# FermiQ/octree-mg

Hardware: AMD Instinct MI355X
Metric: V-cycle cell-updates/s + smoother HBM GB/s vs roofline, 3D Poisson 512^3 (higher is better)
Workload: dtype f64; 1 GPU; C3: 3D Poisson, 512^3 per GPU, box 16, periodic, GSRB FAS V-cycle (n_cycle_down=up=2); mode=weak, box_size=16, parallelism=domain-decomposition x1 (RCCL halos)

## Files before the change

### octree-mg_amd/csrc/omg_tiles.hip

```cpp
#include <stdexcept>
#include <string>

#include "omg_face.h"
#include "omg_gsrb.h"
#include "omg_kernels.h"

namespace omg {

constexpr int kPsBS16 = 512, kPsWaves = 8;
constexpr int kSumsLPW = 32, kSumsR = 4;
constexpr bool kSumsNT = true, kSubNTLd = false, kSubNTSt = false;

template <int NC, int OP, int BS, bool STORE = true>
__device__ __forceinline__ void resid_restrict_core(const LevelView& F, const LevelView& Cv, double lambda,
                                                    unsigned long long* maxbits, int restrict_on,
                                                    const int* parent_local, const int* dixp, int b, double* sb,
                                                    const v2d* fr);

template <int NC, int OP, int BS, bool STORE = true>
__device__ __forceinline__ void resid_restrict_box(const LevelView& F, const LevelView& Cv, double lambda,
                                                   unsigned long long* maxbits, int restrict_on,
                                                   const int* parent_local, const int* dixp, int b, double* sb,
                                                   const double* __restrict__ rsh = nullptr, int n_rsh = 0) {
  using TL = Tl<NC>;
  constexpr int NST = TL::NST, HV = TL::HV, NR = (HV + BS - 1) / BS;
  const int tid = threadIdx.x;
  const long long boff = (long long)b * F.stride;
  const double* __restrict__ u = F.phi + boff;
  const double* __restrict__ f = F.data + F.vstride + boff;
  for (int q = tid; q < NST / 2; q += BS) reinterpret_cast<v2d*>(sb)[q] = ld_nt(u + 2 * q);
  v2d fr[NR];
#pragma unroll
  for (int r = 0; r < NR; r++) {
    const int q2 = tid + BS * r;
    if (q2 < HV) fr[r] = ld_nt(f + 2 * q2);
  }
  if (n_rsh) {
    const RhsSub rsub(rsh, n_rsh);
#pragma unroll
    for (int r = 0; r < NR; r++)
      if (tid + BS * r < HV) {
        double a = fr[r].x, b2 = fr[r].y;
        rsub(a, b2);
        fr[r].x = a;
        fr[r].y = b2;
      }
  }
  __syncthreads();
  resid_restrict_core<NC, OP, BS, STORE>(F, Cv, lambda, maxbits, restrict_on, parent_local, dixp, b, sb, fr);
}

template <bool ON>
__device__ __forceinline__ int step_zero(double mx) {
  if constexpr (ON) {
    int zero = 0;
    asm volatile("" : "+v"(zero) : "v"(mx));
    return zero;
  } else {
    return 0;
  }
}

template <int NC, int OP, int BS, bool STORE>
__device__ __forceinline__ void resid_restrict_core(const LevelView& F, const LevelView& Cv, double lambda,
                                                    unsigned long long* maxbits, int restrict_on,
                                                    const int* parent_local, const int* dixp, int b, double* sb,
                                                    const v2d* fr) {
  using TL = Tl<NC>;
  constexpr int HV = TL::HV, FH = TL::FH, FS = TL::FS, NR = (HV + BS - 1) / BS, HN = NC / 2;
  const int tid = threadIdx.x;
  double* __restrict__ res = F.data + 3 * F.vstride + (long long)b * F.stride;

  const OpCoef<OP> K(F, lambda);
  double mx = 0.0;
  double2 rv[NR];
#pragma unroll
  for (int r = 0; r < NR; r++) {
    const int q2 = tid + BS * r;
    if (q2 >= HV) continue;
    const int e = q2 >= HV / 2, o = 1 - e;
    Nbr7 s0, s1;
    if constexpr (HN % 2 == 0) {
      pair_stencil<NC>(sb + o * HV, sb + 2 * HV + o * FH, FS, e,
                       2 * q2 - e * HV + step_zero<!STORE && (NR > 1)>(mx), s0, s1);
    } else {
      int i, j, k;
      TL::decode(2 * q2, i, j, k);
      s0.xm = sb[TL::ocell(i - 1, j, k)]; s0.xp = sb[TL::ocell(i + 1, j, k)];
      s0.ym = sb[TL::ocell(i, j - 1, k)]; s0.yp = sb[TL::ocell(i, j + 1, k)];
      s0.zm = sb[TL::ocell(i, j, k - 1)]; s0.zp = sb[TL::ocell(i, j, k + 1)];
      TL::decode(2 * q2 + 1, i, j, k);
      s1.xm = sb[TL::ocell(i - 1, j, k)]; s1.xp = sb[TL::ocell(i + 1, j, k)];
      s1.ym = sb[TL::ocell(i, j - 1, k)]; s1.yp = sb[TL::ocell(i, j + 1, k)];
      s1.zm = sb[TL::ocell(i, j, k - 1)]; s1.zp = sb[TL::ocell(i, j, k + 1)];
    }
    const double2 cc = reinterpret_cast<const double2*>(sb)[q2];
    s0.c = cc.x;
    s1.c = cc.y;
    double l0, l1;
    op_pair<NC, OP>(K, F, b, e, 2 * q2 - e * HV, s0, s1, l0, l1);
    const double r0 = fr[r].x - l0, r1 = fr[r].y - l1;
    mx = amax(mx, amax(fabs(r0), fabs(r1)));
    rv[r] = make_double2(r0, r1);
    if constexpr (STORE) st_nt(res + 2 * q2, r0, r1);
  }
  if (maxbits) launch_max<BS>(maxbits, mx);
  if (!restrict_on || parent_local[b] < 0) return;

  const int pb = parent_local[b], dp = dixp[b];
  const int dx = dp & 1023, dy = (dp >> 10) & 1023, dz = dp >> 20;
  const long long poff = (long long)pb * Cv.stride;
  for (int pass = 0; pass < 2; pass++) {
    double* __restrict__ dst = pass == 0 ? Cv.phi + poff : Cv.data + 3 * Cv.vstride + poff;
    for (int q = tid; q < HN * HN * HN; q += BS) {
      const int i = q % HN + 1, j = (q / HN) % HN + 1, k = q / (HN * HN) + 1;
      double acc = 0.0;
#pragma unroll
      for (int kk = 0; kk < 2; kk++)
#pragma unroll
        for (int jj = 0; jj < 2; jj++)
#pragma unroll
          for (int ii = 0; ii < 2; ii++) acc += sb[TL::oint(2 * i - 1 + ii, 2 * j - 1 + jj, 2 * k - 1 + kk)];
      dst[off_int(Cv, dx + i, dy + j, dz + k)] = 0.125 * acc;
    }
    if (pass == 0) {
      __syncthreads();
#pragma unroll
      for (int r = 0; r < NR; r++) {
        const int q2 = tid + BS * r;
        if (q2 < HV) reinterpret_cast<double2*>(sb)[q2] = rv[r];
      }
      __syncthreads();
    }
  }
}

template <int NC, int OP, int BS, bool STORE = true>
__global__ void __launch_bounds__(BS) k_resid_restrict(LevelView F, LevelView Cv, double lambda,
                                                       unsigned long long* maxbits, int restrict_on,
                                                       const int* parent_local, const int* dixp,
                                                       const int* list, const double* __restrict__ rsh,
                                                       int n_rsh) {
  __shared__ double sb[Tl<NC>::NST];
  const int q = xcd_box(blockIdx.x, gridDim.x, F.rev);
  resid_restrict_box<NC, OP, BS, STORE>(F, Cv, lambda, maxbits, restrict_on, parent_local, dixp,
                                        list ? list[q] : q, sb, rsh, n_rsh);
}

template <int NC>
__device__ __forceinline__ int sr_int(int d, int v, int a, int c) {
  return d == 0 ? Tl<NC>::oint(v, a, c) : (d == 1 ? Tl<NC>::oint(a, v, c) : Tl<NC>::oint(a, c, v));
}
template <int NC>
__device__ __forceinline__ int sr_edge(int d, int t, bool lo, int nl, int a, int c) {
  const int t1 = d == 0 ? 1 : 0, t2 = d == 2 ? 1 : 2, ax = t == 0 ? t1 : t2;
  const int fn = 2 * ax + (lo ? 1 : 2);
  const int i = d == 0 ? nl : a, j = d == 1 ? nl : (d == 0 ? a : c), k = d == 2 ? nl : c;
  return ax == 0 ? Tl<NC>::ogh(fn, j, k) : (ax == 1 ? Tl<NC>::ogh(fn, i, k) : Tl<NC>::ogh(fn, i, j));
// ... 433 lines not shown
  }
  __syncthreads();
  const RbSide rbs{Cv, nullptr, rbgv, rbgv ? 1 : 0};
  gsrb_box<NC, OP, BS, 2, true, RB>(F, lambda, 1, 2, bc, nullptr, nullptr, b, lds, nullptr, RB ? &rbs : nullptr);
}

template <int NC, int OP, int BS, bool RB = false>
__global__ void __launch_bounds__(BS, RB ? 4 : kPsWaves) k_prolong_smooth(LevelView Cv, LevelView F, double lambda,
                                                       const int* parent_local, const int* dixp, GcBC bc,
                                                       int one_child, const int* list, const uint8_t* push0,
                                                       double* rbgv) {
  __shared__ double lds[prolong_smooth_lds<NC>()];
  const int t = xcd_box(blockIdx.x, gridDim.x, F.rev);
  prolong_smooth_box<NC, OP, BS, RB>(Cv, F, lambda, parent_local, dixp, bc, one_child, push0, list ? list[t] : t,
                                     lds, rbgv);
}

void launch_prolong_smooth(const LevelView& C, const LevelView& F, int op, double lambda, const int* parent_local,
                           const int* dixp, const GcBC& bc, int one_child, const int* list, int n_list,
                           const uint8_t* push0, hipStream_t st, bool rb, double* rbgv) {
  const int n = list ? n_list : F.n;
  if (n == 0) return;
  const dim3 g(n);
  if (rb) {
    if (F.nc != 16 && F.nc != 8) throw std::runtime_error("launch_prolong_smooth: refinement boundaries need 16^3 / 8^3");
#define OMG_PSR(NC, BS)                                                                                         \
  if (op == OP_HELM)                                                                                            \
    k_prolong_smooth<NC, OP_HELM, BS, true><<<g, BS, 0, st>>>(C, F, lambda, parent_local, dixp, bc, one_child, \
                                                              list, push0, rbgv);                               \
  else                                                                                                          \
    k_prolong_smooth<NC, OP_LPL, BS, true><<<g, BS, 0, st>>>(C, F, lambda, parent_local, dixp, bc, one_child,  \
                                                             list, push0, rbgv);
    if (F.nc == 16) OMG_PSR(16, kPsBS16) else OMG_PSR(8, 256)
#undef OMG_PSR
    return;
  }
#define OMG_PS(NC, BS)                                                                                \
  if (op == OP_HELM)                                                                                  \
    k_prolong_smooth<NC, OP_HELM, BS><<<g, BS, 0, st>>>(C, F, lambda, parent_local, dixp, bc, one_child, \
                                                        list, push0, nullptr);                        \
  else                                                                                                \
    k_prolong_smooth<NC, OP_LPL, BS><<<g, BS, 0, st>>>(C, F, lambda, parent_local, dixp, bc, one_child,  \
                                                       list, push0, nullptr);
  switch (F.nc) {
    case 16: OMG_PS(16, kPsBS16) break;
    case 8: OMG_PS(8, 256) break;
    case 4: OMG_PS(4, 256) break;
    default: OMG_PS(2, 256) break;
  }
#undef OMG_PS
}

template <bool NT>
__device__ __forceinline__ double2 sums_ld(const double* p) {
  if (NT) {
    const v2d t = ld_nt(p);
    return make_double2(t.x, t.y);
  }
  return *reinterpret_cast<const double2*>(p);
}
template <bool NT>
__device__ __forceinline__ void sums_st(double* p, double2 v) {
  if (NT)
    st_nt(p, v.x, v.y);
  else
    *reinterpret_cast<double2*>(p) = v;
}

template <int NC, bool SUB, bool SH = SUB, int LPW = kSumsLPW>
__global__ void __launch_bounds__(64) k_box_sums3(LevelView L, int iv, const int* __restrict__ leaves,
                                                  int n_leaves, double* __restrict__ out,
                                                  const double* __restrict__ shifts, int n_sh) {
  constexpr int H = NC / 2, R = kSumsR < NC ? kSumsR : NC, SEG = R * H;
  constexpr bool NTL = SUB ? kSubNTLd : kSumsNT;
  constexpr int CH2 = SEG;
  constexpr int PER = LPW * CH2 / 64;
  constexpr int P = 2 * SEG + 1;
  constexpr int NCH = NC * NC / R;
  __shared__ double lds[LPW * P];
  const int lane = threadIdx.x, b0 = (L.rev ? gridDim.x - 1 - blockIdx.x : blockIdx.x) * LPW;
  const long long hv = L.hv;
  double* src[PER];
  int dst[PER];
  bool own[PER];
#pragma unroll
  for (int r = 0; r < PER; r++) {
    const int t = lane + 64 * r, bb = t / CH2, w = t % CH2, seg = w / (SEG / 2), off = w % (SEG / 2);
    const int q = min(b0 + bb, n_leaves - 1);
    own[r] = b0 + bb < n_leaves;
    src[r] = boxp(L, iv, leaves[q]) + seg * hv + 2 * off;
    dst[r] = bb * P + seg * SEG + 2 * off;
  }
  static_assert(SH || !SUB, "k_box_sums3: the storing form subtracts");
  const RhsSub rsub(shifts, SH ? n_sh : 0);
  double2 va[PER], vb[PER];
  auto chunk_off = [](int c) { return H * (((c % (NC / R)) * R) + NC * (c / (NC / R))); };
#pragma unroll
  for (int r = 0; r < PER; r++) va[r] = sums_ld<NTL>(src[r]);
#pragma unroll
  for (int r = 0; r < PER; r++) vb[r] = sums_ld<NTL>(src[r] + chunk_off(1));
  double acc = 0.0;
  const double* my = lds + lane * P;
  auto process = [&](double2* v, int c) {
    __syncthreads();
    const int rc = chunk_off(c);
#pragma unroll
    for (int r = 0; r < PER; r++) {
      if (SH) rsub(v[r].x, v[r].y);
      if (SUB && own[r]) sums_st<kSubNTSt>(src[r] + rc, v[r]);
      lds[dst[r]] = v[r].x;
      lds[dst[r] + 1] = v[r].y;
    }
    __syncthreads();
    if (c + 2 < NCH) {
      const int r2 = chunk_off(c + 2);
#pragma unroll
      for (int r = 0; r < PER; r++) v[r] = sums_ld<NTL>(src[r] + r2);
    }
    const int k = c / (NC / R) + 1, j0 = (c % (NC / R)) * R + 1;
    if (lane < LPW) {
#pragma unroll
      for (int rr = 0; rr < R; rr++) {
        const int ca = (1 + j0 + rr + k) & 1;
        const double* A = my + ca * SEG + rr * H;
        const double* B = my + (1 - ca) * SEG + rr * H;
#pragma unroll
        for (int q = 0; q < H; q++) {
          acc += A[q];
          acc += B[q];
        }
      }
    }
  };
  static_assert(NCH % 2 == 0, "chunks come in pairs");
  for (int c = 0; c < NCH; c += 2) {
    process(va, c);
    process(vb, c + 1);
  }
  if (out && lane < LPW && b0 + lane < n_leaves) out[b0 + lane] = acc;
}

__global__ void __launch_bounds__(64) k_box_sums_any(LevelView L, int iv, const int* leaves, int n_leaves,
                                                     double* out) {
  const int q = blockIdx.x * 64 + threadIdx.x;
  if (q >= n_leaves) return;
  const double* u = boxp(L, iv, leaves[q]);
  double acc = 0.0;
  for (int k = 1; k <= L.nc; k++)
    for (int j = 1; j <= L.nc; j++)
      for (int i = 1; i <= L.nc; i++) acc += u[off_int(L, i, j, k)];
  out[q] = acc;
}

__global__ void __launch_bounds__(64) k_seq_sum3(const double* __restrict__ box_sums, int n, double w,
                                                 double* __restrict__ acc, int init) {
  constexpr int CH = 1024, PL = CH / 128, G = 16;
  __shared__ double st[CH];
  const int lane = threadIdx.x;
  double a = init ? 0.0 : *acc;
  double2 pre[PL];
  auto fetch = [&](int base) {
#pragma unroll
    for (int r = 0; r < PL; r++) {
      const int q = base + 2 * (lane + 64 * r);
      pre[r].x = q < n ? box_sums[q] : 0.0;
      pre[r].y = q + 1 < n ? box_sums[q + 1] : 0.0;
    }
  };
  fetch(0);
  for (int base = 0; base < n; base += CH) {
    __syncthreads();
#pragma unroll
    for (int r = 0; r < PL; r++) reinterpret_cast<double2*>(st)[lane + 64 * r] = pre[r];
    __syncthreads();
    if (base + CH < n) fetch(base + CH);
    const int m = min(CH, n - base);
    if (m == CH) {
      double cur[G], nxt[G];
#pragma unroll
      for (int t = 0; t < G; t++) cur[t] = st[t];
      for (int g = 0; g < CH / G; g++) {
        const int gn = g + 1 < CH / G ? g + 1 : g;
#pragma unroll
        for (int t = 0; t < G; t++) nxt[t] = st[G * gn + t];
        double p[G];
#pragma unroll
        for (int t = 0; t < G; t++) p[t] = w * cur[t];
#pragma unroll
        for (int t = 0; t < G; t++) a = a + p[t];
#pragma unroll
        for (int t = 0; t < G; t++) cur[t] = nxt[t];
      }
    } else {
      for (int q = 0; q < m; q++) a = a + w * st[q];
    }
  }
  if (lane == 0) *acc = a;
}

template <int NC, int BS>
__global__ void __launch_bounds__(BS) k_fill_tile(LevelView L, GcBC bc, double* sendbuf) {
  constexpr int HV = Tl<NC>::HV;
  __shared__ double sb[2 * HV];
  const int b = xcd_box(blockIdx.x, gridDim.x, L.rev);
  const FaceTopo T = load_topo(L, b);
  const double* u = L.phi + (long long)b * L.stride;
  for (int q = threadIdx.x; q < HV; q += BS) reinterpret_cast<v2d*>(sb)[q] = reinterpret_cast<const v2d*>(u)[q];
  __syncthreads();
  tile_face_fill<NC>(L, b, T, sb, 3, bc, sendbuf);
}

template <int NC, int BS>
__global__ void __launch_bounds__(BS) k_fill_tile_xl(LevelView L, GcBC bc, double* sendbuf,
                                                     const double* __restrict__ xl) {
  using TL = Tl<NC>;
  constexpr int HV = TL::HV, H = NC / 2, FH = H * NC;
  __shared__ double sb[2 * HV];
  const int b = xcd_box(blockIdx.x, gridDim.x, L.rev);
  const FaceTopo T = load_topo(L, b);
  const double* u = L.phi + (long long)b * L.stride;
  bool phys = false;
#pragma unroll
  for (int nb = 0; nb < 6; nb++) phys |= T.kind(nb) == NB_PHYS;
  if (phys) {
    for (int q = threadIdx.x; q < HV; q += BS) reinterpret_cast<v2d*>(sb)[q] = reinterpret_cast<const v2d*>(u)[q];
  } else {
    const int t = threadIdx.x;
    for (int q = t; q < 2 * FH; q += BS) {
      const int e = q / FH, w = q % FH, pl = w / (FH / 2), r2 = w % (FH / 2);
      const int off = e * HV + (pl ? FH * (NC - 1) : 0) + 2 * r2;
      *reinterpret_cast<v2d*>(sb + off) = *reinterpret_cast<const v2d*>(u + off);
    }
    for (int q = t; q < 4 * NC * (H / 2); q += BS) {
      const int r2 = q % (H / 2), row = q / (H / 2), k = row % NC, jj = (row / NC) & 1, e = row / (2 * NC);
      const int off = e * HV + H * ((jj ? NC - 1 : 0) + NC * k) + 2 * r2;
      *reinterpret_cast<v2d*>(sb + off) = *reinterpret_cast<const v2d*>(u + off);
    }
    const double* xb = xl + (long long)b * 512;
    for (int q = t; q < 2 * NC * NC; q += BS) {
      const int f = q / (NC * NC), c = q % (NC * NC), j = c % NC + 1, k = c / NC + 1;
      sb[TL::oint(f ? NC : 1, j, k)] = xb[q];
    }
  }
  __syncthreads();
  tile_face_fill<NC>(L, b, T, sb, 3, bc, sendbuf);
}

void launch_fill_tile_xl(const LevelView& L, const GcBC& bc, double* sendbuf, const double* xl, hipStream_t st) {
  if (L.n == 0) return;
  if (L.nc != 16) throw std::runtime_error("launch_fill_tile_xl: 16^3 boxes only");
  k_fill_tile_xl<16, 512><<<L.n, 512, 0, st>>>(L, bc, sendbuf, xl);
}

bool launch_fill_tile(const LevelView& L, const GcBC& bc, double* sendbuf, hipStream_t st) {
  if (L.n == 0) return true;
  const dim3 g(L.n);
  switch (L.nc) {
    case 16: k_fill_tile<16, 512><<<g, 512, 0, st>>>(L, bc, sendbuf); return true;
    case 8: k_fill_tile<8, 256><<<g, 256, 0, st>>>(L, bc, sendbuf); return true;
    case 4: k_fill_tile<4, 64><<<g, 64, 0, st>>>(L, bc, sendbuf); return true;
    default: return false;
  }
}

bool launch_smooth_resid(const LevelView& F, const LevelView& C, int op, double lambda, int restrict_on,
                         const int* parent_local, const int* dixp, hipStream_t st, const int* list,
                         int n_list, const GcBC& bc, bool has_rb, bool has_phys, const double* rbgv) {
  if (op != OP_LPL && op != OP_HELM) return false;
  if (!has_rb) rbgv = nullptr;
  const int n = list ? n_list : F.n;
  if (n == 0) return true;
  const dim3 g(n);
#define OMG_SR_RB(NC, BS, RB)                                                                                    \
  if (op == OP_LPL)                                                                                              \
    k_smooth_resid<NC, OP_LPL, BS, RB><<<g, BS, 0, st>>>(F, C, lambda, restrict_on, parent_local, dixp, list, bc,   \
                                                         rbgv);                                                   \
  else                                                                                                           \
    k_smooth_resid<NC, OP_HELM, BS, RB><<<g, BS, 0, st>>>(F, C, lambda, restrict_on, parent_local, dixp, list, bc,  \
                                                          rbgv);
#define OMG_SR(NC, BS)           \
  if (has_rb) {                  \
    OMG_SR_RB(NC, BS, 2)         \
  } else if (has_phys) {         \
    OMG_SR_RB(NC, BS, 1)         \
  } else {                       \
    OMG_SR_RB(NC, BS, 0)         \
  }
  switch (F.nc) {
    case 16: OMG_SR(16, 512) return true;
    case 8: OMG_SR(8, 256) return true;
    default: return false;
  }
#undef OMG_SR
#undef OMG_SR_RB
}

bool tiled_nc(int nc) { return nc == 16 || nc == 8 || nc == 4 || nc == 2; }

void launch_resid_restrict(const LevelView& F, const LevelView& C, int op, double lambda,
                           unsigned long long* maxbits, int restrict_on, const int* parent_local,
                           const int* dixp, hipStream_t st, const int* list, int n_list, RhsShifts rs,
                           bool store) {
  const int n = list ? n_list : F.n;
  if (n == 0) return;
  if (rs.n < 0 || rs.n > kRhsPendMax || (rs.n && !rs.s))
    throw std::runtime_error("launch_resid_restrict: at most kRhsPendMax pending rhs shifts");
  const dim3 g(n);
#define OMG_RR_OP(NC, BS, OPV)                                                                             \
  if (store)                                                                                               \
    k_resid_restrict<NC, OPV, BS, true><<<g, dim3(BS), 0, st>>>(F, C, lambda, maxbits, restrict_on,        \
                                                                parent_local, dixp, list, rs.s, rs.n);     \
  else                                                                                                     \
    k_resid_restrict<NC, OPV, BS, false><<<g, dim3(BS), 0, st>>>(F, C, lambda, maxbits, restrict_on,       \
                                                                 parent_local, dixp, list, rs.s, rs.n);
#define OMG_RR(NC, BS) OMG_FOR_OP(op, OMG_RR_OP, NC, BS)
  switch (F.nc) {
    case 16: OMG_RR(16, 512) break;
    case 8: OMG_RR(8, 256) break;
    case 4: OMG_RR(4, 256) break;
    default: OMG_RR(2, 256) break;
  }
#undef OMG_RR
#undef OMG_RR_OP
}

void launch_prolong_fill(const LevelView& C, const LevelView& F, int iv, const int* parent_local,
                         const int* dixp, const GcBC& bc, double* sendbuf, bool sub, bool skip1,
                         hipStream_t st, const int* list, int n_list, bool save_old, const RBRec* rb) {
  const int n = list ? n_list : F.n;
  if (n == 0) return;
  const dim3 g(n);
  const int so = save_old && !skip1;
#define OMG_PF(NC, BS)                                                                                              \
  if (rb && sub)                                                                                                    \
    k_prolong_fill<NC, BS, true, true><<<g, BS, 0, st>>>(C, F, iv, parent_local, dixp, bc, sendbuf, skip1, list, so, rb); \
  else if (rb)                                                                                                      \
    k_prolong_fill<NC, BS, false, true><<<g, BS, 0, st>>>(C, F, iv, parent_local, dixp, bc, sendbuf, skip1, list, so, rb); \
  else if (sub)                                                                                                     \
    k_prolong_fill<NC, BS, true><<<g, BS, 0, st>>>(C, F, iv, parent_local, dixp, bc, sendbuf, skip1, list, so, rb); \
  else                                                                                                              \
    k_prolong_fill<NC, BS, false><<<g, BS, 0, st>>>(C, F, iv, parent_local, dixp, bc, sendbuf, skip1, list, so, rb);
  switch (F.nc) {
    case 16: OMG_PF(16, 512) break;
    case 8: OMG_PF(8, 256) break;
    case 4: OMG_PF(4, 256) break;
    default: OMG_PF(2, 256) break;
  }
#undef OMG_PF
}

template <int NC, int OP, int BS, bool NT = false>
// ... 79 lines not shown
      sb[TL::ogh(nb, a, c)] = C.phi[(long long)T.arg(f) * C.stride + sr_int<NC>(d, low ? NC : 1, a, c)];
    }
    const double* __restrict__ res = C.data + 3 * C.vstride + boff;
#pragma unroll
    for (int r = 0; r < NR; r++) {
      const int q2 = tid + BS * r;
      if (q2 < HV) rr[r] = ld_nt(res + 2 * q2);
    }
  }
  __syncthreads();
  tile_face_fill<NC>(C, b, T, sb, 3, bc, nullptr);
  if (!par) return;
  if (T.nonlocal()) {
    for (int p = tid; p < 6 * NC * NC; p += BS) {
      const int f = p / (NC * NC), cell = p % (NC * NC);
      if (T.kind(f) != NB_PHYS) continue;
      const int nb = f + 1, a = cell % NC + 1, c = cell / NC + 1, d = f >> 1;
      const bool low = nb & 1;
      const int gi = TL::ogh(nb, a, c);
      sb[gi] = phys_ghost(C, bc, b, (long long)b * 6 + f, nb, T.phys_code(f), a, c, gi,
                          sb[sr_int<NC>(d, low ? 1 : NC, a, c)], sb[sr_int<NC>(d, low ? 2 : NC - 1, a, c)]);
    }
  }
  __syncthreads();
  double* __restrict__ old = C.data + 2 * C.vstride + boff;
  double* __restrict__ rhs = C.data + C.vstride + boff;
  for (int q = tid; q < NST / 2; q += BS) {
    const v2d x = reinterpret_cast<const v2d*>(sb)[q];
    st_nt(old + 2 * q, x.x, x.y);
  }
  const OpCoef<OP> K(C, lambda);
  constexpr int FS = TL::FS;
#pragma unroll
  for (int r = 0; r < NR; r++) {
    const int q2 = tid + BS * r;
    if (q2 >= HV) continue;
    const int e = q2 >= HV / 2, o = 1 - e;
    Nbr7 s0, s1;
    if constexpr (H % 2 == 0) {
      pair_stencil<NC>(sb + o * HV, sb + 2 * HV + o * FH, FS, e, 2 * q2 - e * HV, s0, s1);
    } else {
      int i, j, k;
      TL::decode(2 * q2, i, j, k);
      s0.xm = sb[TL::ocell(i - 1, j, k)]; s0.xp = sb[TL::ocell(i + 1, j, k)];
      s0.ym = sb[TL::ocell(i, j - 1, k)]; s0.yp = sb[TL::ocell(i, j + 1, k)];
      s0.zm = sb[TL::ocell(i, j, k - 1)]; s0.zp = sb[TL::ocell(i, j, k + 1)];
      TL::decode(2 * q2 + 1, i, j, k);
      s1.xm = sb[TL::ocell(i - 1, j, k)]; s1.xp = sb[TL::ocell(i + 1, j, k)];
      s1.ym = sb[TL::ocell(i, j - 1, k)]; s1.yp = sb[TL::ocell(i, j + 1, k)];
      s1.zm = sb[TL::ocell(i, j, k - 1)]; s1.zp = sb[TL::ocell(i, j, k + 1)];
    }
    const double2 cc = reinterpret_cast<const double2*>(sb)[q2];
    s0.c = cc.x;
    s1.c = cc.y;
    double l0, l1;
    op_pair<NC, OP>(K, C, b, e, 2 * q2 - e * HV, s0, s1, l0, l1);
    st_nt(rhs + 2 * q2, l0 + rr[r].x, l1 + rr[r].y);
  }
}

void launch_fill_crhs(const LevelView& C, int op, double lambda, const GcBC& bc, const uint8_t* parmask,
                      hipStream_t st) {
  if (C.n == 0) return;
  const dim3 g(C.n);
#define OMG_FC_OP(NC, BS, OPV) k_fill_crhs<NC, OPV, BS><<<g, BS, 0, st>>>(C, lambda, bc, parmask);
#define OMG_FC(NC, BS) OMG_FOR_OP(op, OMG_FC_OP, NC, BS)
  switch (C.nc) {
    case 16: OMG_FC(16, 512) break;
    case 8: OMG_FC(8, 256) break;
    case 4: OMG_FC(4, 64) break;
    default: throw std::runtime_error("launch_fill_crhs: box sizes 16, 8, 4");
  }
#undef OMG_FC
#undef OMG_FC_OP
}

template <int NC, int OP, int BS>
__global__ void __launch_bounds__(BS) k_coarse_rhs_tile(LevelView Cv, double lambda, const int* parents) {
  __shared__ double sb[Tl<NC>::NST];
  coarse_rhs_box<NC, OP, BS, true>(Cv, lambda, parents[xcd_box(blockIdx.x, gridDim.x, Cv.rev)], sb);
}

bool launch_coarse_rhs_tile(const LevelView& C, int op, double lambda, const int* parents, int n_par,
                            hipStream_t st) {
  if (!tiled_nc(C.nc)) return false;
  if (n_par == 0) return true;
  const dim3 g(n_par);
#define OMG_CR_OP(NC, BS, OPV) k_coarse_rhs_tile<NC, OPV, BS><<<g, BS, 0, st>>>(C, lambda, parents);
#define OMG_CR(NC, BS) OMG_FOR_OP(op, OMG_CR_OP, NC, BS)
  switch (C.nc) {
    case 16: OMG_CR(16, 512) break;
    case 8: OMG_CR(8, 256) break;
    case 4: OMG_CR(4, 256) break;
    default: OMG_CR(2, 256) break;
  }
#undef OMG_CR
#undef OMG_CR_OP
  return true;
}

static void check_shifts(const RhsShifts& rs, const char* who) {
  if (rs.n < 0 || rs.n > kRhsPendMax + 1 || (rs.n && !rs.s))
    throw std::runtime_error(std::string(who) + ": at most kRhsPendMax + 1 shifts");
}

void launch_box_sums(const LevelView& L, int iv, const int* leaves, int n, double* out, hipStream_t st,
                     RhsShifts rs) {
  if (n == 0) return;
  check_shifts(rs, "launch_box_sums");
  if (rs.n && !subtract_sums_nc(L.nc)) throw std::runtime_error("launch_box_sums: shifts need a 16 / 8 / 4 box");
  const dim3 g((n + kSumsLPW - 1) / kSumsLPW);
  switch (L.nc) {
#define OMG_BS(NC)                                                                         \
  if (rs.n) k_box_sums3<NC, false, true><<<g, 64, 0, st>>>(L, iv, leaves, n, out, rs.s, rs.n); \
  else k_box_sums3<NC, false, false><<<g, 64, 0, st>>>(L, iv, leaves, n, out, nullptr, 0);
    case 16: OMG_BS(16) break;
    case 8: OMG_BS(8) break;
    case 4: OMG_BS(4) break;
#undef OMG_BS
    default: k_box_sums_any<<<(n + 63) / 64, 64, 0, st>>>(L, iv, leaves, n, out); break;
  }
}

bool subtract_sums_nc(int nc) { return nc == 16 || nc == 8 || nc == 4; }

void launch_subtract_sums(const LevelView& L, int iv, const int* leaves, int n, RhsShifts rs, double* out,
                          hipStream_t st) {
  if (n == 0) return;
  check_shifts(rs, "launch_subtract_sums");
  const dim3 g((n + kSumsLPW - 1) / kSumsLPW);
  switch (L.nc) {
    case 16: k_box_sums3<16, true><<<g, 64, 0, st>>>(L, iv, leaves, n, out, rs.s, rs.n); break;
    case 8: k_box_sums3<8, true><<<g, 64, 0, st>>>(L, iv, leaves, n, out, rs.s, rs.n); break;
    case 4: k_box_sums3<4, true><<<g, 64, 0, st>>>(L, iv, leaves, n, out, rs.s, rs.n); break;
    default: throw std::runtime_error("launch_subtract_sums: box size must be 16, 8 or 4");
  }
}

__global__ void k_mean(const double* all, int n, double volume, double* mean) {
  __shared__ double t[64];
  if (threadIdx.x || blockIdx.x) return;
  for (int r = 0; r < n; r++) t[r] = all[r];
  for (int w = 1; w < n; w *= 2)
    for (int r = 0; r + w < n; r += 2 * w) t[r] = t[r] + t[r + w];
  *mean = t[0] / volume;
}

void launch_mean(const double* all, int n, double volume, double* mean, hipStream_t st) {
  k_mean<<<1, 64, 0, st>>>(all, n, volume, mean);
}

void launch_seq_sum(const double* box_sums, int n, double w, double* acc, bool init, hipStream_t st) {
  if (n == 0) return;
  k_seq_sum3<<<1, 64, 0, st>>>(box_sums, n, w, acc, init);
}

constexpr int kTailBS = 512;
template <bool LEX>
constexpr int tail_lds() {
  return LEX && gs_lex_lds<16>() > Tl<16>::NST ? gs_lex_lds<16>() : Tl<16>::NST;
}

__device__ void tail_fill(const TailArgs& A, int li);

template <int OP, bool LEX>
__device__ void tail_smooth(const TailArgs& A, int li, int n_cycle, double* lds) {
  const TailLevel& T = A.lv[li];
  if constexpr (LEX) {
    for (int n = 1; n <= n_cycle; n++) {
      for (int b = 0; b < T.L.n; b++) {
        switch (T.L.nc) {
          case 16: gs_lex_box<OP, 16>(T.L, A.lambda, b, lds); break;
          case 8: gs_lex_box<OP, 8>(T.L, A.lambda, b, lds); break;
          case 4: gs_lex_box<OP, 4>(T.L, A.lambda, b, lds); break;
          default: gs_lex_box<OP, 2>(T.L, A.lambda, b, lds); break;
        }
      }
      tail_fill(A, li);
    }
    return;
  }
  for (int n = 1; n <= 2 * n_cycle; n++) {
    const int e = n & 1;
    for (int b = 0; b < T.L.n; b++) {
      switch (T.L.nc) {
        case 16: gsrb_box<16, OP, kTailBS, 0>(T.L, A.lambda, e, 1 << e, T.bc, nullptr, nullptr, b, lds); break;
        case 8: gsrb_box<8, OP, kTailBS, 0>(T.L, A.lambda, e, 1 << e, T.bc, nullptr, nullptr, b, lds); break;
        case 4: gsrb_box<4, OP, kTailBS, 0>(T.L, A.lambda, e, 1 << e, T.bc, nullptr, nullptr, b, lds); break;
        default: gsrb_box<2, OP, kTailBS, 0>(T.L, A.lambda, e, 1 << e, T.bc, nullptr, nullptr, b, lds); break;
      }
      __syncthreads();
    }
  }
}

template <int OP>
__device__ double tail_residual(const TailArgs& A, int li, int restrict_on, bool want_max, double* lds) {
  const TailLevel& T = A.lv[li];
  const LevelView C = restrict_on ? A.lv[li - 1].L : T.L;
  unsigned long long* mb = want_max ? A.maxbits : nullptr;
  if (want_max) {
    if (threadIdx.x == 0) *mb = 0ull;
    __syncthreads();
  }
  for (int b = 0; b < T.L.n; b++) {
    switch (T.L.nc) {
      case 16: resid_restrict_box<16, OP, kTailBS>(T.L, C, A.lambda, mb, restrict_on, T.parent_local, T.dixp, b, lds); break;
      case 8: resid_restrict_box<8, OP, kTailBS>(T.L, C, A.lambda, mb, restrict_on, T.parent_local, T.dixp, b, lds); break;
      case 4: resid_restrict_box<4, OP, kTailBS>(T.L, C, A.lambda, mb, restrict_on, T.parent_local, T.dixp, b, lds); break;
      default: resid_restrict_box<2, OP, kTailBS>(T.L, C, A.lambda, mb, restrict_on, T.parent_local, T.dixp, b, lds); break;
    }
    __syncthreads();
  }
  if (!want_max) return 0.0;
  const unsigned long long bits = __hip_atomic_load(mb, __ATOMIC_RELAXED, __HIP_MEMORY_SCOPE_WORKGROUP);
  __syncthreads();
  return __longlong_as_double((long long)bits);
}

__device__ void tail_fill(const TailArgs& A, int li) {
  const TailLevel& T = A.lv[li];
  const int nc = T.L.nc, nc2 = nc * nc;
  const LevelView none{};
  if (nc == 1) {
    for (int b = threadIdx.x; b < T.L.n; b += blockDim.x) box1_fill(T.L, 1, b, none, nullptr, T.bc, nullptr);
  } else {
    for (int t = threadIdx.x; t < T.L.n * 6 * nc2; t += blockDim.x) {
      const int cell = t % nc2, f = t / nc2;
      face_cell_fill(T.L, 1, f / 6, f % 6 + 1, cell % nc + 1, cell / nc + 1, 3, none, nullptr, T.bc, nullptr);
    }
  }
  __syncthreads();
}

template <int OP>
__device__ void tail_coarse_rhs(const TailArgs& A, int li, double* lds) {
  const TailLevel& T = A.lv[li];
  for (int p = 0; p < T.n_par; p++) {
    const int b = T.parents[p];
    switch (T.L.nc) {
      case 16: coarse_rhs_box<16, OP, kTailBS>(T.L, A.lambda, b, lds); break;
      case 8: coarse_rhs_box<8, OP, kTailBS>(T.L, A.lambda, b, lds); break;
      case 4: coarse_rhs_box<4, OP, kTailBS>(T.L, A.lambda, b, lds); break;
      default: coarse_rhs_box<2, OP, kTailBS>(T.L, A.lambda, b, lds); break;
    }
    __syncthreads();
  }
}

__device__ void tail_correct(const TailArgs& A, int li, double* lds) {
  const TailLevel& T = A.lv[li];
  const LevelView C = A.lv[li - 1].L;
  for (int b = 0; b < T.L.n; b++) {
    switch (T.L.nc) {
      case 16: prolong_fill_box<16, kTailBS, true>(C, T.L, 4, T.parent_local, T.dixp, T.bc, nullptr, b, lds, false); break;
      case 8: prolong_fill_box<8, kTailBS, true>(C, T.L, 4, T.parent_local, T.dixp, T.bc, nullptr, b, lds, false); break;
      case 4: prolong_fill_box<4, kTailBS, true>(C, T.L, 4, T.parent_local, T.dixp, T.bc, nullptr, b, lds, false); break;
      default: prolong_fill_box<2, kTailBS, true>(C, T.L, 4, T.parent_local, T.dixp, T.bc, nullptr, b, lds, false); break;
    }
    __syncthreads();
  }
}

constexpr int kTailLdsLevels = kTailLdsMaxLevels;
constexpr int kTailLdsDoubles = 4 * (10 * 10 * 10 + 6 * 6 * 6 + 4 * 4 * 4);
constexpr int kTailLdsBcDoubles = 6 * (8 * 8 + 4 * 4 + 2 * 2);
constexpr int kTailBigS = 18, kTailBigS3 = kTailBigS * kTailBigS * kTailBigS;
constexpr int kTailBigDoubles = 2 * kTailBigS3 + 6 * 16 * 16;

struct TailBox {
  double *P, *F, *O, *R;
  double* B;
  int nc, S;
  int ln;
  __device__ __forceinline__ int at(int i, int j, int k) const { return i + S * (j + S * k); }
};

__device__ __forceinline__ Nbr7 tail_nbr(const TailBox& X, const double* U, int c) {
  Nbr7 s;
  s.c = U[c];
  s.xm = U[c - 1];
  s.xp = U[c + 1];
  s.ym = U[c - X.S];
  s.yp = U[c + X.S];
  s.zm = U[c - X.S * X.S];
  s.zp = U[c + X.S * X.S];
  return s;
}

struct TailLdsLevel {
  int local[6];
  double c0[6], c1[6], c2[6];
};

__device__ __forceinline__ TailBox tail_box(const TailArgs& A, int li, double* tl) {
  TailBox X;
  int base = 0, bbase = kTailLdsDoubles;
  for (int l = 0; l < li; l++) {
    const int s = A.lv[l].L.nc + 2;
    base += 4 * s * s * s;
    bbase += 6 * A.lv[l].L.nc * A.lv[l].L.nc;
  }
  X.nc = A.lv[li].L.nc;
  X.S = X.nc + 2;
  X.ln = 31 - __clz(X.nc);
  const int s3 = X.S * X.S * X.S;
  X.P = tl + base;
// ... 719 lines not shown
```

Before: 39.45 billion cell-updates/s.

## Warp-specialize sequential sum: producer waves prefetch into double-buffered LDS

Rewrites the single-wave ordered summation kernel so one wave runs the serial add chain while three extra waves fetch the next chunk, pre-multiply by w, and stage it into a double-buffered shared array. The aim is to take global loads, LDS staging and multiplies off the latency-bound serial dependency chain. Inline asm fences keep the summation order fixed so results stay deterministic. It adds barriers per chunk and more threads. The kernel runs once per sum, so its share of total V-cycle time is probably small.

```diff
diff --git a/octree-mg_amd/csrc/omg_seqsum.h b/octree-mg_amd/csrc/omg_seqsum.h
--- /dev/null
+++ b/octree-mg_amd/csrc/omg_seqsum.h
@@ -0,0 +1,84 @@
+#pragma once
+#include <hip/hip_runtime.h>
+
+namespace omg {
+
+constexpr int kSeqCH = 1024, kSeqBS = 256, kSeqG = 16;
+
+__device__ __forceinline__ void seq_fence(double& a) { asm volatile("" : "+v"(a) : : "memory"); }
+static_assert(kSeqG == 16, "seq_arrived names the eight reads of a group");
+__device__ __forceinline__ void seq_arrived(double2 (&v)[kSeqG / 2]) {
+  asm volatile(""
+               : "+v"(v[0].x), "+v"(v[1].x), "+v"(v[2].x), "+v"(v[3].x), "+v"(v[4].x), "+v"(v[5].x), "+v"(v[6].x),
+                 "+v"(v[7].x));
+}
+
+__global__ void __launch_bounds__(kSeqBS) k_seq_sum3(const double* __restrict__ box_sums, int n, double w,
+                                                     double* __restrict__ acc, int init) {
+  constexpr int CH = kSeqCH, G = kSeqG, NP = kSeqBS - 64, PL = (CH / 2 + NP - 1) / NP;
+  __shared__ double2 st[2][CH / 2];
+  const int tid = threadIdx.x, pt = tid - 64;
+  const bool chain = tid < 64, prep = !chain;
+  double a = 0.0;
+  if (chain && !init) a = *acc;
+  double2 pre[PL];
+  auto fetch = [&](int base) {
+#pragma unroll
+    for (int r = 0; r < PL; r++) {
+      const int i = pt + NP * r, q = base + 2 * i;
+      if (i < CH / 2) {
+        pre[r].x = q < n ? w * box_sums[q] : 0.0;
+        pre[r].y = q + 1 < n ? w * box_sums[q + 1] : 0.0;
+      }
+    }
+  };
+  auto stage = [&](int s) {
+#pragma unroll
+    for (int r = 0; r < PL; r++)
+      if (pt + NP * r < CH / 2) st[s][pt + NP * r] = pre[r];
+  };
+  if (prep) {
+    fetch(0);
+    stage(0);
+    if (CH < n) fetch(CH);
+  }
+  __syncthreads();
+  int s = 0;
+  for (int base = 0; base < n; base += CH, s ^= 1) {
+    if (chain) {
+      const int m = __builtin_amdgcn_readfirstlane(min(CH, n - base)), ng = m / G;
+      const double2* p = st[s];
+      double2 A[G / 2], B[G / 2];
+      auto group = [&](double2* v, int g) {
+        const int gc = g < CH / G ? g : CH / G - 1;
+#pragma unroll
+        for (int t = 0; t < G / 2; t++) v[t] = p[(G / 2) * gc + t];
+        seq_fence(a);
+      };
+      auto add = [&](double2 (&v)[G / 2]) {
+        seq_arrived(v);
+#pragma unroll
+        for (int t = 0; t < G / 2; t++) {
+          a = a + v[t].x;
+          a = a + v[t].y;
+        }
+      };
+      group(A, 0);
+      for (int g = 0; g < ng; g += 2) {
+        group(B, g + 1);
+        add(A);
+        group(A, g + 2);
+        if (g + 1 < ng) add(B);
+      }
+      const double* pd = reinterpret_cast<const double*>(p);
+      for (int q = ng * G; q < m; q++) a = a + pd[q];
+    } else if (base + CH < n) {
+      stage(s ^ 1);
+      if (base + 2 * CH < n) fetch(base + 2 * CH);
+    }
+    __syncthreads();
+  }
+  if (tid == 0) *acc = a;
+}
+
+}
diff --git a/octree-mg_amd/csrc/omg_tiles.hip b/octree-mg_amd/csrc/omg_tiles.hip
--- a/octree-mg_amd/csrc/omg_tiles.hip
+++ b/octree-mg_amd/csrc/omg_tiles.hip
@@ -4,6 +4,7 @@
 #include "omg_face.h"
 #include "omg_gsrb.h"
 #include "omg_kernels.h"
+#include "omg_seqsum.h"
 
 namespace omg {
 
@@ -743,51 +744,6 @@
   out[q] = acc;
 }
 
-__global__ void __launch_bounds__(64) k_seq_sum3(const double* __restrict__ box_sums, int n, double w,
-                                                 double* __restrict__ acc, int init) {
-  constexpr int CH = 1024, PL = CH / 128, G = 16;
-  __shared__ double st[CH];
-  const int lane = threadIdx.x;
-  double a = init ? 0.0 : *acc;
-  double2 pre[PL];
-  auto fetch = [&](int base) {
-#pragma unroll
-    for (int r = 0; r < PL; r++) {
-      const int q = base + 2 * (lane + 64 * r);
-      pre[r].x = q < n ? box_sums[q] : 0.0;
-      pre[r].y = q + 1 < n ? box_sums[q + 1] : 0.0;
-    }
-  };
-  fetch(0);
-  for (int base = 0; base < n; base += CH) {
-    __syncthreads();
-#pragma unroll
-    for (int r = 0; r < PL; r++) reinterpret_cast<double2*>(st)[lane + 64 * r] = pre[r];
-    __syncthreads();
-    if (base + CH < n) fetch(base + CH);
-    const int m = min(CH, n - base);
-    if (m == CH) {
-      double cur[G], nxt[G];
-#pragma unroll
-      for (int t = 0; t < G; t++) cur[t] = st[t];
-      for (int g = 0; g < CH / G; g++) {
-        const int gn = g + 1 < CH / G ? g + 1 : g;
-#pragma unroll
-        for (int t = 0; t < G; t++) nxt[t] = st[G * gn + t];
-        double p[G];
-#pragma unroll
-        for (int t = 0; t < G; t++) p[t] = w * cur[t];
-#pragma unroll
-        for (int t = 0; t < G; t++) a = a + p[t];
-#pragma unroll
-        for (int t = 0; t < G; t++) cur[t] = nxt[t];
-      }
-    } else {
-      for (int q = 0; q < m; q++) a = a + w * st[q];
-    }
-  }
-  if (lane == 0) *acc = a;
-}
 
 template <int NC, int BS>
 __global__ void __launch_bounds__(BS) k_fill_tile(LevelView L, GcBC bc, double* sendbuf) {
@@ -1173,7 +1129,7 @@
 
 void launch_seq_sum(const double* box_sums, int n, double w, double* acc, bool init, hipStream_t st) {
   if (n == 0) return;
-  k_seq_sum3<<<1, 64, 0, st>>>(box_sums, n, w, acc, init);
+  k_seq_sum3<<<1, kSeqBS, 0, st>>>(box_sums, n, w, acc, init);
 }
 
 constexpr int kTailBS = 512;
```

Measured after the change: 39.68 billion cell-updates/s, median of 6. Within noise of the previous version (+0.6%).
